# sinhvt3421/scann--material

Hardware: AMD Instinct MI355X
Metric: QM9 molecules/s forward (higher is better)
Workload: dtype f32 (projections: split-fp16 hi/lo operands, 3 v_mfma_f32_32x32x16_f16 per product, fp32 accumulate; everything else fp32)

## Files before the change

scann--material_amd/csrc/scann_edge_body.inc:

```
  _Float16* const sH = reinterpret_cast<_Float16*>(sTile);
  _Float16* const sL = sH + TEK * PLANE_STRIDE;
  float* const sK = reinterpret_cast<float*>(sTile);

  const int tid = threadIdx.x, lane = tid & 63, wave = tid >> 6;
  const int tix = SCANN_EDGE_TIX;
  const EdgeTile tile = a.tiles[tix];
  const int part = a.tile_part ? a.tile_part[tix] : -1;
  const int eb = tile.edge_begin, ne = tile.edge_end - eb, natom = tile.atom_end - tile.atom_begin;
  const int nem1 = ne > 0 ? ne - 1 : 0;
  const bool live = ne > 0;
  const int lrow = lane & 31, lh = lane >> 5;
  const int cbase = 32 * wave + 4 * lh;
  const int blk_jstride = 8 * ne;
  const auto blk_off = [&](int rt) __attribute__((always_inline)) {
    return ((unsigned)eb * D + ((unsigned)(8 * wave + lh) * ne + min(lrow + 32 * rt, nem1)) * 4) * 4;
  };

  STAMP(a.stamps, 0);
  STAMP_IF(a.stamps, 6, threadIdx.x == 0 && eb >= 0);
  STAMP_HWID(a.stamps, 14);
  STAMP_REAL(a.stamps, 12);
  WRegs<EX> wr;
  f16x8 fth[2], ftl[2];
  if (GUPD) {
    if (!FB) {
      load_whalf<EX>(wr, a.p.W2h, wave, lane, 0);
      __builtin_amdgcn_sched_barrier(0);
    }
  } else {
    load_wsplit<2>(a.p.Wfh, wave, lane, fth, ftl);
  }
  unsigned nboff[RT];
  int ctr[RT];
  float ewgt[RT] = {};
  const int32_t* const ecol = live ? a.edge_col : a.edge_offset;
  const int32_t* const erow = live ? a.edge_row : a.edge_offset;
#pragma unroll
  for (int rt = 0; rt < RT; ++rt) {
    const unsigned e4 = live ? (unsigned)(eb + min(lrow + 32 * rt, nem1)) * 4u : 0u;
    const int nbr = ld1i(ecol, e4), crw = ld1i(erow, e4);
    int nb = live ? nbr : 0;
    if (FB && a.species) nb = ld1i(a.species, (unsigned)nb * 4u);
    nboff[rt] = ((unsigned)nb * D + cbase) * 4;
    ctr[rt] = live ? crw - tile.atom_begin : 0;
    if (!GUPD) {
      const float wv = ld1f(live ? a.edge_weight : reinterpret_cast<const float*>(a.edge_offset), e4);
      ewgt[rt] = live ? wv : 0.f;
    }
  }
  const int voff = ld1i(a.edge_offset, (unsigned)(tile.atom_begin + min(tid, natom)) * 4u);
  STAMP_IF(a.stamps, 10, threadIdx.x == 0 && nboff[0] != 0xfffffff1u);
  const float bkc = a.p.bk[tid & (D - 1)];
  const float par0 = GUPD ? (tid < D ? a.p.lng_g : a.p.lng_b)[tid & (D - 1)] : a.p.bfg[tid & (D - 1)];
  const float par1 = (tid < D ? a.p.ln_g : a.p.ln_b)[tid & (D - 1)];
  float4 greg[RT][4];
  {
    const int r = tid >> 2, sub = tid & 3;
    const int rs = r < ne ? r : nem1;
    if (GUPD) {
      float4 p1reg[3];
#pragma unroll
      for (int i = 0; i < 3; ++i) {
        const int idx = tid + 256 * i, la = min(idx >> 5, natom - 1), c4 = idx & 31;
        const int arow = FB && a.species ? a.species[tile.atom_begin + la] : tile.atom_begin + la;
        p1reg[i] = ld4(a.P1, ((unsigned)arow * 32 + c4) * 16);
      }
      if (FB) {
        _Float16* const bH = reinterpret_cast<_Float16*>(sTile);
        _Float16* const bL = bH + TEK * BASIS_STRIDE;
        f16x8 bdh[2], bdl[2], bwh[2], bwl[2];
        load_wsplit<2>(a.basis.Wdh, wave, lane, bdh, bdl);
        load_wsplit<2>(a.basis.Wwh, wave, lane, bwh, bwl);
        {
          const float xd = ne > 0 ? a.dist[eb + rs] : 0.f, xw = ne > 0 ? a.edge_weight[eb + rs] : 0.f;
// ... 396 lines not shown
```

scann--material_amd/csrc/scann_forward.cpp:

```cpp
#include "scann_runtime.h"

namespace {

constexpr unsigned kTimingEventFlags = hipEventDisableSystemFence;

int ensure_debug(scann_handle* h, scann_dbatch* db) {
  const int L = h->cfg.n_attention;
  if (db->dbg_layers == L) return SCANN_OK;
  HIPCHK(h, cached_malloc((void**)&db->dbg_c, (size_t)(L + 1) * db->n_atom * D * 4));
  HIPCHK(h, cached_malloc((void**)&db->dbg_ctx, (size_t)std::max(L, 1) * db->n_atom * D * 4));
  if (h->cfg.g_update) HIPCHK(h, cached_malloc((void**)&db->dbg_g, (size_t)(L + 1) * std::max(db->n_edge, 1) * D * 4));
  db->dbg_layers = L;
  return SCANN_OK;
}

int ensure_outputs(scann_handle* h, scann_dbatch* db, bool infer) {
  db->out_layers = infer ? h->out_layers : 0;
  db->out_flags = infer ? h->out_flags : 0;
  db->out_attn = db->out_z = db->out_bf = nullptr;
  if (!db->out_layers && !db->out_flags) return SCANN_OK;
  const scann_config_t& c = h->cfg;
  const size_t n_attn = (size_t)__builtin_popcountll(db->out_layers) * db->n_edge * c.num_head;
  const size_t n_z = db->out_flags & SCANN_OUT_AFTER_LC ? (size_t)db->n_atom * c.global_dim : 0;
  const size_t n_bf = db->out_flags & SCANN_OUT_BF_PROPERTY ? (size_t)db->n_struct * c.dense_out : 0;
// ... 325 lines not shown
    }
#endif
    if (exact) {
      a.exact = 1;
      if (l > 0 && a.ffn) {
        const LayerParams& pp = W->layers[l - 1];
        a.Wf1h = reinterpret_cast<const _Float16*>(pp.Wf1p); a.Wf2h = reinterpret_cast<const _Float16*>(pp.Wf2p);
      }
      if (l < L) {
        const LayerParams& p = W->layers[l];
        a.WAh = reinterpret_cast<const _Float16*>(p.W1p); a.WBh = reinterpret_cast<const _Float16*>(p.W3p);
        a.WCh = reinterpret_cast<const _Float16*>(p.Wqp);
      } else {
        a.WAh = reinterpret_cast<const _Float16*>(W->head.Wap); a.WCh = reinterpret_cast<const _Float16*>(W->head.Wgqp);
        a.WDh = reinterpret_cast<const _Float16*>(W->head.Wgkp);
      }
    }
    if (!(species0 && l == 0)) launch_atom(a, s);
    if (tm) tm->mark(l < L ? 1 : 3);
    if (l == L) break;
    EdgeArgs ea{};
    ea.tiles = db->tiles; ea.n_tile = db->n_tile; ea.g_update = c.g_update; ea.tile_rows = db->tile_rows;
    ea.edge_offset = db->edge_offset; ea.edge_col = db->edge_col; ea.edge_row = db->edge_row;
    ea.geom = g_of(l); ea.geom_out = debug && c.g_update ? g_of(l + 1) : nullptr; ea.gd = b.gd; ea.edge_weight = db->weight;
    if (fuse_basis && l == 0) { ea.fuse_basis = 1; ea.dist = db->dist; ea.basis = W->basis; }
    ea.n_edge = db->n_edge;
    ea.geom_rows = fuse_basis ? 0 : 1;
    ea.geom_dead = (l == L - 1 && !debug) ? 1 : 0;
    ea.c = c_of(l); ea.P1 = b.P1; ea.P3 = b.P3; ea.q = keep ? db->keep_q + (size_t)l * nA_ : b.q; ea.ctx = ctx_of(l);
    ea.n_member = nm; ea.m_w = wst; ea.m_a = ea.m_r = ast;
    if (species0 && l == 0) { ea.species = db->atomic; ea.c = W->sp_c; ea.P1 = W->sp_P1; ea.P3 = W->sp_P3; ea.q = W->sp_q; ea.m_r = wst; }
    if (keep) {
      ea.keep_V = db->keep_V + (size_t)l * nE_; ea.keep_K = db->keep_K + (size_t)l * nE_;
      if (db->keep_T) ea.keep_T = db->keep_T + (size_t)l * nE_;
      if (db->keep_ang) ea.keep_ang = db->keep_ang + (size_t)l * nE_;
      db->kept = true;
    }
    ea.p = W->layers[l];
    if (exact) {
      ea.exact = 1;
      ea.p.W2h = reinterpret_cast<const _Float16*>(ea.p.W2p); ea.p.Wkh = reinterpret_cast<const _Float16*>(ea.p.Wkp);
    }
    ea.range_flag = rflag; ea.layer = l;
    const bool sample = !tm && !mc && !o.of_set && h->time_every > 0 && (h->time_count % h->time_every) == 0 && !(fuse_basis && l == 0) &&
                        !(ea.geom_dead && L > 2);
    hipEvent_t ev0 = nullptr, ev1 = nullptr;
    if (sample) {
      (void)hipEventCreateWithFlags(&ev0, kTimingEventFlags);
      (void)hipEventCreateWithFlags(&ev1, kTimingEventFlags);
      (void)hipEventRecord(ev0, s);
    }
    ea.tile_part = db->tile_part; ea.part_buf = b.part_buf;
    ea.xcd_remap = h->xcd_remap;
    ea.attn_out = o.outputs ? attn_out_of(h, db, l) : nullptr;
    if (tr && tr->attn_p > 0.f) {
      ea.attn_drop_p = tr->attn_p;
      ea.attn_drop_seed = tr->seed;
      ea.attn_drop_tag = DROP_TAG_ATTN + (unsigned)l;
    }
    if (mc && mc->p_attn > 0.f && db->n_edge > 0) {
      ea.attn_drop_p = mc->p_attn;
      ea.attn_drop_seed = mc->seed;
      ea.attn_drop_tag = DROP_TAG_ATTN + (unsigned)l;
      ea.mc_rows = mc->rows;
      ea.mc_t = mc->t;
    }
#ifdef SCANN_STAMPS
    if (!getenv("SCANN_STAMP_ATOM") && l == (getenv("SCANN_STAMP_LAYER") ? atoi(getenv("SCANN_STAMP_LAYER")) : L - 1)) {
      if (!db->stamps) HIPCHK(h, hipMalloc((void**)&db->stamps, (size_t)db->n_tile * 16 * sizeof(unsigned long long)));
      ea.stamps = db->stamps;
      db->n_stamp = db->n_tile;
    }
#endif
    launch_edge(ea, s);
    if (nm) launch_edge_merge_set(db->big_tab, db->n_big, b.part_buf, ea.q, ea.p.ln_g, ea.p.ln_b, ea.ctx, rflag, l, nm, ast, wst, s);
    else launch_edge_merge(db->big_tab, db->n_big, b.part_buf, ea.q, ea.p.ln_g, ea.p.ln_b, ea.ctx, rflag, l, s);
    if (ea.attn_out) launch_attn_merge(db->big_tab, db->n_big, b.part_buf, db->edge_offset, db->tile_rows, ea.attn_out, s);
    if (sample) {
      (void)hipEventRecord(ev1, s);
      h->time_ev.push_back(ev0);
      h->time_ev.push_back(ev1);
      h->time_edges.push_back(db->n_edge);
    }
    if (tm) tm->mark(2);
  }
  if (!tm && !mc && !o.of_set) h->time_count++;
  ReadoutArgs r{};
  r.mol_offset = db->mol_offset; r.n_struct = db->n_struct; r.max_atoms = db->max_atoms;
  r.gq = b.gq; r.gk = b.gk; r.use_ga_norm = c.use_ga_norm; r.relu_out = W->cfg.relu_out;
  for (int m = 1; m < nm; ++m) r.relu_out |= o.members[m]->cfg.relu_out << m;
  r.p = W->head; r.ga_attn = b.ga; r.y = b.y; r.bf_out = o.outputs ? db->out_bf : nullptr;
  r.n_member = nm; r.m_w = wst; r.m_a = ast; r.m_g = o.m_g; r.m_y = o.m_y;
  launch_readout(r, s);
  if (tm) tm->mark(3);
  HIPCHK(h, hipGetLastError());
  return SCANN_OK;
}

}

extern "C" {

int scann_forward_resident(scann_handle_t* h, scann_dbatch_t* db, int stream_slot) {
  if (!h || !db) return fail(h, SCANN_ERR_INVALID, "scann_forward_resident: null argument");
  HIPCHK(h, hipSetDevice(h->device));
  const int slot = ((stream_slot % h->nstream) + h->nstream) % h->nstream;
// ... 221 lines not shown
```

scann--material_amd/csrc/scann_internal.h:

```cpp
#pragma once
#include <hip/hip_runtime.h>
#include <stdint.h>

#include <string>
#include <vector>

namespace scann {

constexpr int D = 128;
constexpr int NHEAD = 8;
constexpr int HDIM = D / NHEAD;
constexpr int NG = 20;
constexpr int LDS_STRIDE = 132;
constexpr int TE_MAX = 64;
constexpr int TA = 64;
constexpr int TQ = 24;
constexpr int WPACK = D * D;
constexpr float WSCALE = 256.f;
constexpr float WMAX = 65504.f / WSCALE;

__host__ __device__ inline float drop_scale(unsigned long long seed, unsigned tag, size_t idx, float p) {
  unsigned long long z = seed + 0x9E3779B97F4A7C15ull * (idx + 1) + ((unsigned long long)tag << 48);
  z = (z ^ (z >> 30)) * 0xBF58476D1CE4E5B9ull;
  z = (z ^ (z >> 27)) * 0x94D049BB133111EBull;
// ... 84 lines not shown

void launch_basis(const BasisParams& p, const float* dist, const float* weight, int n_edge,
                  float* geom, hipStream_t s);
void launch_basis_raw(const float* cd, const float* dist, int n_edge, float* gd, hipStream_t s);

struct EmbedArgs {
  int32_t n_atom, emb_dim;
  const int32_t* atomic;
  const float* cgcnn;
  const float* ring;
  const float *emb;
  const float *We, *be;
  const float *Wr, *br;
  const float *Wde, *bde;
  float* c0;
};
void launch_embed(const EmbedArgs& a, hipStream_t s);

struct AtomArgs {
  const float* x;
  const int32_t* x_index;
  int32_t n_atom;
  int32_t ffn;
  const _Float16 *Wf1h, *Wf2h;
  const float *bf1, *bf2, *lnr_g, *lnr_b;
  float* c;
  float drop_p;
  uint32_t drop_tag;
  unsigned long long drop_seed;
  int32_t mode;
  const _Float16 *WAh, *WBh, *WCh, *WDh;
  const float *bA;
  const float *bC;
  const float *bD;
  float *oA, *oB, *oC;
  float *keep_pre1, *keep_H1, *keep_T2;
  float *keep_preA, *keep_z;
  unsigned long long* stamps;
  int32_t* range_flag;
  int32_t layer;
  int32_t exact;
  float* out_z;
  const McRow* mc_rows;
  uint32_t mc_t;
  int32_t n_member;
  int64_t m_w, m_x, m_o;
};
void launch_atom(const AtomArgs& a, hipStream_t s);

struct EdgeArgs {
  const EdgeTile* tiles;
  int32_t n_tile;
  int32_t xcd_remap;
  const int32_t* tile_part;
  float* part_buf;
  int32_t g_update;
  const int32_t* edge_offset;
  const int32_t* edge_col;
  const int32_t* edge_row;
  float* geom;
  float *keep_V, *keep_T, *keep_ang, *keep_K;
  float* geom_out;
  int32_t tile_rows;
  int32_t n_edge;
  int32_t geom_rows;
  int32_t geom_dead;
  const float* gd;
  const float* edge_weight;
  int32_t fuse_basis;
  const int32_t* species;
  const float* dist;
  BasisParams basis;
  const float *c, *P1, *P3, *q;
  float* ctx;
  float attn_drop_p;
  uint32_t attn_drop_tag;
  unsigned long long attn_drop_seed;
  unsigned long long* stamps;
  int32_t* range_flag;
  int32_t layer;
  int32_t exact;
  LayerParams p;
  float* attn_out;
  const McRow* mc_rows;
  uint32_t mc_t;
  int32_t n_member;
  int64_t m_w, m_r, m_a;
};
void launch_edge(const EdgeArgs& a, hipStream_t s);
void launch_attn_merge(const int32_t* big_tab, int n_big, const float* part_buf, const int32_t* edge_offset, int chunk, float* attn, hipStream_t s);
void launch_edge_merge(const int32_t* big_tab, int n_big, const float* part_buf, const float* q, const float* ln_g,
                       const float* ln_b, float* ctx, int32_t* range_flag, int layer, hipStream_t s);
void launch_edge_merge_set(const int32_t* big_tab, int n_big, const float* part_buf, const float* q, const float* ln_g, const float* ln_b,
                           float* ctx, int32_t* range_flag, int layer, int n_member, int64_t m_a, int64_t m_w, hipStream_t s);

struct GenSeg {
  const float* p;
  const int32_t* idx;
  int32_t w;
};
struct GenDenseArgs {
  GenSeg seg[3];
  int32_t n_seg;
  int32_t prod;
  const float* W;
  const float* b;
// ... 132 lines not shown
```

scann--material_amd/csrc/scann_kernels.hip:

```cpp
#include <algorithm>
#include <cstdlib>
#include <type_traits>
#include "scann_internal.h"
#include "scann_mma.h"

namespace scann {


__device__ __forceinline__ void mc_row_key(const AtomArgs& a, int atom, unsigned long long& seed, size_t& e) {
  const McRow m = a.mc_rows[atom];
  seed = mc_seed(a.drop_seed, a.mc_t, m.key);
  e = (size_t)(atom - m.a0) * D;
}
__device__ __forceinline__ float4 mc_drop4(unsigned long long seed, unsigned tag, size_t e, float p, float4 v) {
  v.x *= drop_scale(seed, tag, e, p);
  v.y *= drop_scale(seed, tag, e + 1, p);
  v.z *= drop_scale(seed, tag, e + 2, p);
  v.w *= drop_scale(seed, tag, e + 3, p);
  return v;
}
__device__ __forceinline__ float4 mc_keep4(uint32_t bits, float p, float4 v) {
  const float sc = 1.0f / (1.0f - p);
  v.x *= (bits & 1u) ? sc : 0.f;
  v.y *= (bits & 2u) ? sc : 0.f;
// ... 113 lines not shown
  } else {
    if (a.mode == 0) SCANN_ATOM_CASE(false, 0);
    else if (a.mode == 1) SCANN_ATOM_CASE(false, 1);
    else SCANN_ATOM_CASE(false, 2);
  }
#undef SCANN_ATOM_CASE
}


template <bool GUPD, int RT, bool FB = false, bool EX = false, bool KEEP = false, bool DEAD = false, bool ATTN = false, bool MC = false,
          bool SET = false>
__global__ __launch_bounds__(256, RT == 2 ? 3 : 4) void edge_kernel(EdgeArgs a) {
#pragma clang fp contract(off)
  static_assert(!FB || GUPD, "the fused basis exists for the g_update kernel only");
  static_assert(!(FB && EX), "the exact fallback runs the plain first layer");
  static_assert(!KEEP || (!FB && !EX && !DEAD), "the training forward runs the plain split-fp16 kernel and keeps every layer's geometry");
  static_assert(!DEAD || GUPD, "the base branch stores no geometry");
  static_assert(!(ATTN && KEEP), "the training forward returns no attention weights");
  static_assert(!MC || (!EX && !KEEP && !ATTN), "Monte Carlo dropout runs on the split-fp16 inference kernels and returns no attention weights");
  static_assert(!SET || (!EX && !KEEP && !ATTN && !MC), "a model set runs the split-fp16 inference kernels and returns no attention weights");
  constexpr int TEK = 32 * RT;
  constexpr bool BLK = GUPD && !EX && !KEEP;
  __shared__ __attribute__((aligned(16))) unsigned char sTile[2 * TEK * PLANE_STRIDE * 2];
  __shared__ __attribute__((aligned(16))) float sQ[TQ * LDS_STRIDE];
  __shared__ __attribute__((aligned(16))) float sE[NHEAD * (TEK + 1)];
#ifdef SCANN_DIAG_SE_ROWMAJOR
#define SE_STAT(w, r) (((r) * 4 + (w)) * 2)
#define SE_LOGIT(r, h) ((r) * NHEAD + (h))
#else
#define SE_STAT(w, r) (((w) * TEK + (r)) * 2)
#define SE_LOGIT(r, h) ((h) * (TEK + 1) + (r))
#endif
  __shared__ __attribute__((aligned(16))) float sPar[5 * D];
  __shared__ int sOff[TQ + 1];
#ifdef SCANN_DIAG_OCC2
  __shared__ float sDummy[7 * 1024];
  if (a.n_tile < 0) sDummy[threadIdx.x] = 1.f;
#endif
  static_assert(2 * TEK * PLANE_STRIDE * 2 >= TEK * LDS_STRIDE * (int)sizeof(float), "K tile must fit the plane buffer");
  int set_tix = 0;
  if constexpr (SET) {
    const int t = a.xcd_remap ? xcd_tile(blockIdx.x, gridDim.x) : blockIdx.x, m = t / a.n_tile;
    set_tix = t - m * a.n_tile;
    const int64_t w = (int64_t)m * a.m_w, r = (int64_t)m * a.m_r, x = (int64_t)m * a.m_a;
    a.p.W2h = set_member(a.p.W2h, w); a.p.Wkh = set_member(a.p.Wkh, w); a.p.Wfh = set_member(a.p.Wfh, w);
    a.p.bfg = set_member(a.p.bfg, w); a.p.bk = set_member(a.p.bk, w);
    a.p.lng_g = set_member(a.p.lng_g, w); a.p.lng_b = set_member(a.p.lng_b, w); a.p.ln_g = set_member(a.p.ln_g, w); a.p.ln_b = set_member(a.p.ln_b, w);
    a.basis.Wdh = set_member(a.basis.Wdh, w); a.basis.Wwh = set_member(a.basis.Wwh, w); a.basis.bd = set_member(a.basis.bd, w);
    a.basis.bw = set_member(a.basis.bw, w); a.basis.cd = set_member(a.basis.cd, w); a.basis.cw = set_member(a.basis.cw, w);
    a.c = set_member(a.c, r); a.P1 = set_member(a.P1, r); a.P3 = set_member(a.P3, r); a.q = set_member(a.q, r);
    a.geom = set_member(a.geom, x); a.ctx = set_member(a.ctx, x); a.part_buf = set_member(a.part_buf, x);
  }
#define SCANN_EDGE_TIX (SET ? set_tix : a.xcd_remap ? xcd_tile(blockIdx.x, gridDim.x) : blockIdx.x)
#include "scann_edge_body.inc"
#undef SCANN_EDGE_TIX
#undef SE_STAT
#undef SE_LOGIT
#ifdef SCANN_DIAG_TAILWAIT
  __builtin_amdgcn_s_waitcnt(0);
  __syncthreads();
#endif
}

template <bool SET = false>
__global__ __launch_bounds__(128) void edge_merge_kernel(const int32_t* __restrict__ big_tab, const float* __restrict__ part_buf,
                                                         const float* __restrict__ q, const float* __restrict__ ln_g,
                                                         const float* __restrict__ ln_b, float* __restrict__ ctx,
                                                         int32_t* __restrict__ range_flag, int layer, int n_big, int64_t m_a, int64_t m_w) {
  __shared__ float sRed[2][2];
  unsigned bix = blockIdx.x;
  if constexpr (SET) {
    const unsigned m = blockIdx.x / (unsigned)n_big;
    bix = blockIdx.x - m * (unsigned)n_big;
    part_buf = set_member(part_buf, (int64_t)m * m_a); q = set_member(q, (int64_t)m * m_a); ctx = set_member(ctx, (int64_t)m * m_a);
    ln_g = set_member(ln_g, (int64_t)m * m_w); ln_b = set_member(ln_b, (int64_t)m * m_w);
  }
  const int c = threadIdx.x, atom = big_tab[3 * bix], s0 = big_tab[3 * bix + 1], ns = big_tab[3 * bix + 2];
  const float* pb = part_buf + (size_t)s0 * 3 * D + c;
  float M = -INFINITY;
  for (int i = 0; i < ns; ++i) M = fmaxf(M, pb[(size_t)i * 3 * D]);
  float S = 0.f, X = 0.f;
  for (int i = 0; i < ns; ++i) {
    const float wgt = fast_exp(pb[(size_t)i * 3 * D] - M);
    S += pb[(size_t)i * 3 * D + D] * wgt;
    X += pb[(size_t)i * 3 * D + 2 * D] * wgt;
  }
  const float t = X * __builtin_amdgcn_rcpf(S) + q[(size_t)atom * D + c];
  float s = t;
#pragma unroll
  for (int o = 1; o < 64; o <<= 1) s += __shfl_xor(s, o);
  if ((c & 63) == 0) sRed[0][c >> 6] = s;
  __syncthreads();
  const float mean = (sRed[0][0] + sRed[0][1]) * (1.0f / D);
  const float d = t - mean;
  float v = d * d;
#pragma unroll
  for (int o = 1; o < 64; o <<= 1) v += __shfl_xor(v, o);
  if ((c & 63) == 0) sRed[1][c >> 6] = v;
  __syncthreads();
  if (!(sRed[1][0] + sRed[1][1] < RANGE_FINITE) && c == 0) flag_range(range_flag, 2, layer);
  const float rstd = ln_rstd((sRed[1][0] + sRed[1][1]) * (1.0f / D));
  ctx[(size_t)atom * D + c] = ln_apply(t, rstd, -mean * rstd, ln_g[c], ln_b[c]);
}

void launch_edge_merge(const int32_t* big_tab, int n_big, const float* part_buf, const float* q, const float* ln_g,
                       const float* ln_b, float* ctx, int32_t* range_flag, int layer, hipStream_t s) {
  if (n_big > 0)
    hipLaunchKernelGGL(edge_merge_kernel<false>, dim3(n_big), dim3(128), 0, s, big_tab, part_buf, q, ln_g, ln_b, ctx, range_flag, layer, n_big,
                       (int64_t)0, (int64_t)0);
}
void launch_edge_merge_set(const int32_t* big_tab, int n_big, const float* part_buf, const float* q, const float* ln_g, const float* ln_b,
                           float* ctx, int32_t* range_flag, int layer, int n_member, int64_t m_a, int64_t m_w, hipStream_t s) {
  if (n_big > 0 && n_member > 0)
    hipLaunchKernelGGL(edge_merge_kernel<true>, dim3(n_big * n_member), dim3(128), 0, s, big_tab, part_buf, q, ln_g, ln_b, ctx, range_flag, layer,
// ... 14 lines not shown
    const float mi = pb[(size_t)(n / chunk) * 3 * D];
    float* const w = attn + (size_t)(e0 + n) * NHEAD + h;
    *w = *w * fast_exp(mi - M) * __builtin_amdgcn_rcpf(S);
  }
}

void launch_attn_merge(const int32_t* big_tab, int n_big, const float* part_buf, const int32_t* edge_offset, int chunk, float* attn, hipStream_t s) {
  if (n_big > 0 && attn) hipLaunchKernelGGL(attn_merge_kernel, dim3(n_big), dim3(256), 0, s, big_tab, part_buf, edge_offset, chunk, attn);
}

__global__ void edge_row_kernel(const int32_t* __restrict__ edge_offset, int n_atom, int32_t* __restrict__ edge_row, int32_t* __restrict__ zero_word) {
  const int a = blockIdx.x * blockDim.x + threadIdx.x;
  if (a == 0 && zero_word) *zero_word = 0;
  if (a >= n_atom) return;
  for (int e = edge_offset[a]; e < edge_offset[a + 1]; ++e) edge_row[e] = a;
}
void launch_edge_row(const int32_t* edge_offset, int n_atom, int32_t* edge_row, hipStream_t s, int32_t* zero_word) {
  if (n_atom > 0 || zero_word)
    hipLaunchKernelGGL(edge_row_kernel, dim3(std::max(1, (n_atom + 255) / 256)), dim3(256), 0, s, edge_offset, n_atom, edge_row, zero_word);
}

__global__ __launch_bounds__(256) void pack_padded_kernel(PackPaddedArgs a) {
  const int bm = blockIdx.x * blockDim.x + threadIdx.x;
  if (bm >= a.B * a.M) return;
  const int row = a.row_of[bm];
  if (row < 0) return;
  const int z = a.atomic[bm];
  int bad = (z < 0 || z >= a.n_species) ? 2 : 0;
  a.out_atomic[row] = bad ? 0 : z;
  const int b0 = (bm / a.M) * a.M;
  int e = a.edge_offset[row];
  const size_t base = (size_t)bm * a.N;
  for (int n = 0; n < a.N; ++n) {
    const bool on = a.mask_size == 1 ? static_cast<const uint8_t*>(a.neighbor_mask)[base + n] != 0
                                     : (static_cast<const uint32_t*>(a.neighbor_mask)[base + n] & 0x7fffffffu) != 0;
    if (!on) continue;
    const int tgt = a.neighbors[base + n];
    const int r = (tgt >= 0 && tgt < a.M) ? a.row_of[b0 + tgt] : -1;
    if (r < 0) bad |= 1;
    a.out_col[e] = r < 0 ? row : r;
    a.out_dist[e] = a.dist[base + n];
    a.out_weight[e] = a.weight[base + n];
    ++e;
  }
  if (bad) atomicOr(a.flag, bad);
}
void launch_pack_padded(const PackPaddedArgs& a, hipStream_t s) {
  const int n = a.B * a.M;
  if (n > 0) hipLaunchKernelGGL(pack_padded_kernel, dim3((n + 255) / 256), dim3(256), 0, s, a);
}

void launch_edge(const EdgeArgs& a, hipStream_t s) {
  if (a.n_tile <= 0) return;
  const dim3 grid(a.n_tile * std::max(a.n_member, 1)), block(256);
  const bool keep = !a.exact && (a.geom_rows || a.keep_V || a.keep_T || a.keep_ang || a.keep_K || a.attn_drop_p > 0.f);
  const bool dead = a.g_update && a.geom_dead && !keep;
#define SCANN_EDGE_GO(...) hipLaunchKernelGGL((edge_kernel<__VA_ARGS__>), grid, block, 0, s, a)
#define SCANN_EDGE_ROWS(G, ...)                                             \
  do {                                                                      \
    if (a.tile_rows == 32) SCANN_EDGE_GO(G, 1, __VA_ARGS__);                \
    else SCANN_EDGE_GO(G, 2, __VA_ARGS__);                                  \
  } while (0)
  if (a.n_member > 0) {
    if (!a.g_update) SCANN_EDGE_ROWS(false, false, false, false, false, false, false, true);
    else if (a.fuse_basis) SCANN_EDGE_ROWS(true, true, false, false, false, false, false, true);
    else if (a.geom_dead) SCANN_EDGE_ROWS(true, false, false, false, true, false, false, true);
    else SCANN_EDGE_ROWS(true, false, false, false, false, false, false, true);
  } else if (a.mc_rows && a.attn_drop_p > 0.f) {
    if (!a.g_update) SCANN_EDGE_ROWS(false, false, false, false, false, false, true);
    else if (a.fuse_basis) SCANN_EDGE_ROWS(true, true, false, false, false, false, true);
    else if (a.geom_dead) SCANN_EDGE_ROWS(true, false, false, false, true, false, true);
    else SCANN_EDGE_ROWS(true, false, false, false, false, false, true);
  } else if (a.exact && a.attn_out) {
    if (!a.g_update) SCANN_EDGE_ROWS(false, false, true, false, false, true);
    else if (dead) SCANN_EDGE_ROWS(true, false, true, false, true, true);
    else SCANN_EDGE_ROWS(true, false, true, false, false, true);
  } else if (a.exact) {
    if (!a.g_update) SCANN_EDGE_ROWS(false, false, true, false, false);
    else if (dead) SCANN_EDGE_ROWS(true, false, true, false, true);
    else SCANN_EDGE_ROWS(true, false, true, false, false);
  } else if (a.attn_out) {
    if (!a.g_update) SCANN_EDGE_ROWS(false, false, false, false, false, true);
    else if (a.fuse_basis) SCANN_EDGE_ROWS(true, true, false, false, false, true);
    else if (a.geom_dead) SCANN_EDGE_ROWS(true, false, false, false, true, true);
    else SCANN_EDGE_ROWS(true, false, false, false, false, true);
  } else if (keep) {
    if (a.g_update) SCANN_EDGE_ROWS(true, false, false, true, false);
    else SCANN_EDGE_ROWS(false, false, false, true, false);
  } else if (!a.g_update) {
    SCANN_EDGE_ROWS(false, false, false, false, false);
  } else if (a.fuse_basis) {
    SCANN_EDGE_ROWS(true, true, false, false, false);
  } else {
    if (dead) SCANN_EDGE_ROWS(true, false, false, false, true);
    else SCANN_EDGE_ROWS(true, false, false, false, false);
  }
#undef SCANN_EDGE_ROWS
#undef SCANN_EDGE_GO
}


__global__ __launch_bounds__(256) void basis_kernel(BasisParams p, const float* __restrict__ dist,
                                                    const float* __restrict__ weight, int n_edge,
                                                    float* __restrict__ geom) {
#pragma clang fp contract(off)
  __shared__ __attribute__((aligned(16))) _Float16 sH[64 * BASIS_STRIDE];
  __shared__ __attribute__((aligned(16))) _Float16 sL[64 * BASIS_STRIDE];
  const int tid = threadIdx.x, lane = tid & 63, wave = tid >> 6;
  const int lrow = lane & 31, lh = lane >> 5, cbase = 32 * wave + 4 * lh;
  const int e0 = blockIdx.x * 64;
  const int ne = min(64, n_edge - e0);
  f16x8 bdh[2], bdl[2], bwh[2], bwl[2];
  load_wsplit<2>(p.Wdh, wave, lane, bdh, bdl);
  load_wsplit<2>(p.Wwh, wave, lane, bwh, bwl);
  float4 bd[4], bw[4];
#pragma unroll
  for (int j = 0; j < 4; ++j) {
    bd[j] = *reinterpret_cast<const float4*>(p.bd + cbase + 8 * j);
    bw[j] = *reinterpret_cast<const float4*>(p.bw + cbase + 8 * j);
  }
  {
    const int r = tid >> 2, sub = tid & 3;
    const int rs = min(r, ne - 1);
    const float xd = dist[e0 + rs], xw = weight[e0 + rs];
    f16x8 gh[2], gl[2];
#pragma unroll
    for (int i = 0; i < 8; ++i) {
      const int k = 8 * sub + i;
      const float cdk = p.cd[min(k, NG - 1)], cwk = p.cw[min(k, NG - 1)];
      const float vd = (k < NG && r < ne) ? gauss_fast(xd, cdk) : 0.f, vw = (k < NG && r < ne) ? gauss_fast(xw, cwk) : 0.f;
      gh[0][i] = (_Float16)vd; gl[0][i] = (_Float16)(vd - (float)gh[0][i]);
      gh[1][i] = (_Float16)vw; gl[1][i] = (_Float16)(vw - (float)gh[1][i]);
    }
    *reinterpret_cast<f16x8*>(sH + r * BASIS_STRIDE + 8 * sub) = gh[0];
    *reinterpret_cast<f16x8*>(sL + r * BASIS_STRIDE + 8 * sub) = gl[0];
    *reinterpret_cast<f16x8*>(sH + r * BASIS_STRIDE + 32 + 8 * sub) = gh[1];
    *reinterpret_cast<f16x8*>(sL + r * BASIS_STRIDE + 32 + 8 * sub) = gl[1];
  }
  __syncthreads();
  f32x16 accd[2], accw[2];
  mma_split<2, true, BASIS_STRIDE>(sH, sL, bdh, bdl, lane, accd);
  mma_split<2, true, BASIS_STRIDE>(sH + 32, sL + 32, bwh, bwl, lane, accw);
  constexpr float WINV = 1.0f / WSCALE;
// ... 260 lines not shown
```

scann--material_amd/csrc/scann_runtime.cpp:

```cpp
#include "scann_runtime.h"

#include <mutex>

namespace {

struct BlockCache {
  std::multimap<size_t, void*> free_blocks;
  std::map<void*, size_t> size_of;
  size_t cached_bytes = 0;
};
std::map<int, BlockCache> g_block_cache;
std::mutex g_block_mu;
constexpr size_t BLOCK_CACHE_LIMIT = (size_t)16 << 30;
thread_local std::string g_create_error;

std::vector<WeightSpec> build_specs(const scann_config_t& c) {
  std::vector<WeightSpec> s;
  const int64_t d = c.local_dim, dg = c.global_dim, dout = c.dense_out, emb = c.embedding_dim;
  if (c.feature_cgcnn) {
    s.push_back({"embed_atom/kernel", 92, emb});
    s.push_back({"embed_atom/bias", emb, 0});
  } else {
    s.push_back({"embed_atom/embeddings", c.n_atoms, emb});
  }
// ... 188 lines not shown
    for (int s = 0; s < ks; ++s)
      for (int lane = 0; lane < 64; ++lane)
        for (int j = 0; j < 8; ++j) {
          const int k = 16 * s + 8 * (lane >> 5) + j;
          const float x = k < k_real ? WSCALE * W[(size_t)k * ld + 32 * w + (lane & 31)] : 0.f;
          const uint16_t hi = f32_to_f16_bits(x);
          const uint16_t lo = f32_to_f16_bits(x - f16_bits_to_f32(hi));
          const size_t base = ((size_t)(w * ks + s) * 2) * 64 * 8 + (size_t)lane * 8 + j;
          out[base] = hi;
          out[base + 64 * 8] = lo;
        }
}

}

extern "C" {

int scann_abi_version(void) { return SCANN_ABI_VERSION; }

int scann_device_count(void) {
  int n = 0;
  if (hipGetDeviceCount(&n) != hipSuccess) return 0;
  return n;
}

const char* scann_last_error(const scann_handle_t* h) { return h ? h->err.c_str() : g_create_error.c_str(); }

int scann_create(const scann_config_t* cfg, int device_id, scann_handle_t** out) {
  if (!cfg || !out) return fail(nullptr, SCANN_ERR_INVALID, "scann_create: null argument");
  *out = nullptr;
  if (cfg->n_gauss != NG) return fail(nullptr, SCANN_ERR_UNSUPPORTED, "scann_create: 20 Gaussians (custom_layers.py:39-53 as called by scann_model.py:378,384)");
  const bool generic = cfg->local_dim != D || cfg->global_dim != D || cfg->dense_out != D || cfg->num_head != NHEAD ||
                       (getenv("SCANN_GENERIC") && atoi(getenv("SCANN_GENERIC")));
  if (generic) {
    if (cfg->local_dim <= 0 || cfg->num_head <= 0 || cfg->global_dim <= 0 || cfg->dense_out <= 0 || cfg->local_dim % cfg->num_head != 0)
      return fail(nullptr, SCANN_ERR_INVALID, "scann_create: local_dim must be a positive multiple of num_head (attention.py:170-173), global_dim and dense_out positive");
    if (cfg->local_dim > 1024 || cfg->global_dim > 1024 || cfg->dense_out > 1024 || cfg->embedding_dim > 1024)
      return fail(nullptr, SCANN_ERR_UNSUPPORTED, "scann_create: widths above 1024 are not implemented");
  } else if (cfg->embedding_dim + (cfg->use_ring ? 10 : 0) > 160) {
    return fail(nullptr, SCANN_ERR_UNSUPPORTED, "scann_create: embedding_dim (+10 ring features) must be <= 160");
  }
  if (cfg->n_atoms <= 0 || cfg->embedding_dim <= 0 || cfg->n_attention < 0 || !(cfg->gaussian_d > 0))
    return fail(nullptr, SCANN_ERR_INVALID, "scann_create: bad hyper-parameter");
  int ndev = 0;
  if (hipGetDeviceCount(&ndev) != hipSuccess || ndev <= 0)
    return fail(nullptr, SCANN_ERR_NO_DEVICE, "scann_create: no HIP device visible (this library has no CPU fallback)");
  if (device_id < 0 || device_id >= ndev) return fail(nullptr, SCANN_ERR_NO_DEVICE, "scann_create: device_id out of range");
  scann_handle* h = new scann_handle();
  h->cfg = *cfg;
  h->generic = generic;
  h->device = device_id;
  h->specs = build_specs(*cfg);
  if (const char* xr = getenv("SCANN_XCD_REMAP")) h->xcd_remap = atoi(xr) != 0;
  if (const char* fb = getenv("SCANN_FUSE_BASIS")) h->fuse_basis = atoi(fb) != 0;
  if (const char* st = getenv("SCANN_SPECIES_TABLES")) h->species_tables = atoi(st) != 0;
  if (const char* sg = getenv("SCANN_STRICT_RANGE")) h->strict_range = atoi(sg) != 0;
  if (const char* fe = getenv("SCANN_EXACT")) h->force_exact = atoi(fe) != 0;
  {
    hipDeviceProp_t prop;
    if (hipGetDeviceProperties(&prop, device_id) == hipSuccess && prop.multiProcessorCount > 0) h->n_cu = prop.multiProcessorCount;
  }
  if (const char* ns = getenv("SCANN_STREAMS")) h->nstream = std::min(MAX_STREAM, std::max(1, atoi(ns)));
  if (hipSetDevice(device_id) != hipSuccess) {
    delete h;
    return fail(nullptr, SCANN_ERR_HIP, "scann_create: hipSetDevice failed");
  }
  if (hipHostMalloc((void**)&h->range_flag, 128, hipHostMallocDefault) != hipSuccess) {
    delete h;
    return fail(nullptr, SCANN_ERR_HIP, "scann_create: hipHostMalloc failed");
  }
  for (int i = 0; i < 32; ++i) h->range_flag[i] = 0;
  for (int i = 0; i < h->nstream; ++i) {
    if (hipStreamCreateWithFlags(&h->streams[i], hipStreamNonBlocking) != hipSuccess) {
      delete h;
      return fail(nullptr, SCANN_ERR_HIP, "scann_create: hipStreamCreate failed");
    }
  }
  *out = h;
  return SCANN_OK;
}

void scann_destroy(scann_handle_t* h) {
  if (!h) return;
  (void)hipSetDevice(h->device);
  (void)hipDeviceSynchronize();
  for (int i = 0; i < MAX_STREAM; ++i)
    if (h->streams[i]) (void)hipStreamDestroy(h->streams[i]);
  if (h->d_weights) (void)hipFree(h->d_weights);
  for (scann_handle::DlStage& st : h->dl_stage)
    if (st.p) (void)hipHostFree(st.p);
  if (h->g_weights) (void)hipFree(h->g_weights);
  if (h->g_centres) (void)hipFree(h->g_centres);
  if (h->g_WT) (void)hipFree(h->g_WT);
  if (h->d_gt_descs) (void)hipFree(h->d_gt_descs);
  if (h->sp_c) (void)hipFree(h->sp_c);
  for (scann_handle::Stage& st : h->stage) {
    if (st.p) (void)hipHostFree(st.p);
    if (st.ev) (void)hipEventDestroy(st.ev);
  }
  if (h->copy_stream) (void)hipStreamDestroy(h->copy_stream);
  for (void* q : {(void*)h->t_master, (void*)h->t_grad, (void*)h->t_m, (void*)h->t_v, (void*)h->t_l2, (void*)h->t_descs, (void*)h->ig_grad})
    if (q) (void)hipFree(q);
  if (h->comm) ncclCommDestroy(h->comm);
  if (h->train_aux && !h->train_aux_borrowed) (void)hipStreamDestroy(h->train_aux);
  if (h->h_stat) (void)hipHostFree(h->h_stat);
  if (h->range_flag) (void)hipHostFree(h->range_flag);
// ... 358 lines not shown
```

scann--material_amd/csrc/scann_runtime.h:

```cpp
#pragma once
#include "../../include/scann_hip.h"
#include "scann_internal.h"
#include "scann_train.h"

#include <rccl/rccl.h>

#include <algorithm>
#include <cmath>
#include <cstdlib>
#include <cstring>
#include <map>
#include <memory>
#include <string>
#include <vector>

using namespace scann;

namespace scann {

constexpr int MAX_STREAM = 16;

hipError_t cached_malloc(void** p, size_t bytes);
void cached_free(void* p);
void cache_release(int dev);
// ... 36 lines not shown
  float *keep_preA = nullptr, *keep_z = nullptr;
  std::vector<float*> tE;
  float *rep = nullptr, *dpre = nullptr, *dy = nullptr, *targets = nullptr, *dlut = nullptr;
  float* wpart = nullptr;
  size_t wpart_floats = 0;
  float* det_part = nullptr;
  size_t det_floats = 0;
  double* sse = nullptr;
  char* ig = nullptr;
  size_t ig_bytes = 0;
  float drop_p = 0.f, attn_p = 0.f;
  unsigned long long seed = 0;
  GenKeep gen;
  ~scann_train_ws() {
    cached_free(arena);
    cached_free(det_part);
    cached_free(ig);
    cached_free(gen.arena);
    cached_free(gen.barena);
  }
};

struct Timer;
struct ModelSet;
void free_models(ModelSet* ms);

struct McState {
  const McRow* rows;
  unsigned long long seed;
  uint32_t t;
  float p_drop, p_attn;
};

}

struct scann_handle {
  scann_config_t cfg{};
  int device = 0;
  std::string err;
  hipStream_t streams[MAX_STREAM]{};
  int nstream = 2;
  std::vector<WeightSpec> specs;
  bool loaded = false;
  bool debug = false;
  uint64_t out_layers = 0;
  int32_t out_flags = 0;
  int tile_atoms = TQ;
  int n_cu = 256;
  int time_every = 0;
  int64_t time_count = 0;
  std::vector<hipEvent_t> time_ev;
  std::vector<int> time_edges;
  int xcd_remap = 1;
  int fuse_basis = 1;
  int species_tables = 1;
  bool generic = false;
  float* g_weights = nullptr;
  float* g_centres = nullptr;
  std::map<std::string, int64_t> g_off;
  std::vector<GenTransDesc> gt_descs;
  GenTransDesc* d_gt_descs = nullptr;
  std::map<std::string, int64_t> gt_off;
  float* g_WT = nullptr;
  int gt_max = 0;
  bool weights_exact = false;
  bool force_exact = false;
  bool strict_range = false;
  int64_t exact_reruns = 0;
  float* d_weights = nullptr;
  std::vector<LayerParams> layers;
  HeadParams head{};
  BasisParams basis{};
  const float* lut = nullptr;
  float *sp_c = nullptr, *sp_P1 = nullptr, *sp_P3 = nullptr, *sp_q = nullptr;
  bool sp_dirty = true;
  const float* cd = nullptr;
  EmbedArgs embed{};
  std::vector<float> host_master;
  std::vector<int64_t> spec_off;
  std::vector<RepackDesc> descs;
  size_t arena_floats = 0, o_lut = 0, o_emb = 0, o_Wde = 0, o_bde = 0;
  struct LayerT {
    const float *W1T, *W2T, *W3T, *WqT, *WkT, *Wf1T, *Wf2T;
    const _Float16 *W1Th, *W2Th, *W3Th, *WqTh, *WkTh, *Wf1Th, *Wf2Th;
  };
  std::vector<LayerT> layersT;
  const float *WaT = nullptr, *WgqT = nullptr, *WgkT = nullptr;
  const _Float16* WaTh = nullptr;
  float *t_master = nullptr, *t_grad = nullptr, *t_m = nullptr, *t_v = nullptr, *t_l2 = nullptr;
  RepackDesc* t_descs = nullptr;
  float* ig_grad = nullptr;
  int64_t t_step = 0;
  float attn_drop_p = 0.f;
  bool deterministic = false;
  ncclComm_t comm = nullptr;
  double* h_stat = nullptr;
  float* h_targets[3] = {nullptr, nullptr, nullptr};
  size_t h_targets_cap[3] = {0, 0, 0};
  hipEvent_t step_ev[2] = {nullptr, nullptr};
  int64_t step_begun = 0, step_ended = 0;
  bool grads_zeroed = false;
  struct Stage { char* p = nullptr; size_t cap = 0; hipEvent_t ev = nullptr; bool used = false; };
  static constexpr int N_STAGE = 8;
  Stage stage[N_STAGE];
  int stage_next = 0;
  struct PadScratch { std::vector<int32_t> gidx, at, mol, eoff, col; std::vector<float> dist, wgt, ga; };
// ... 137 lines not shown
```

Baseline: 2.022 million.

## Process edge tiles in pairs per block to cut per-block launch overhead

Adds an edge_pair_kernel that loops over two consecutive edge tiles per workgroup for the bulk of tiles, with the remainder handled one tile per block. The aim is to amortise block startup costs such as weight-register loads and kernarg reads, and to cut wave-launch overhead across the grid. The pair count is rounded to a multiple of three blocks per CU. In exchange, per-block work becomes serial and the added inter-tile __syncthreads may reduce latency hiding. It also relies on the asm barriers (fresh_tid, fresh_edge_args) to keep register pressure in check. The path is enabled by default for 64-row tiles with g_update.

```diff
diff --git a/scann--material_amd/csrc/scann_edge_body.inc b/scann--material_amd/csrc/scann_edge_body.inc
--- a/scann--material_amd/csrc/scann_edge_body.inc
+++ b/scann--material_amd/csrc/scann_edge_body.inc
@@ -2,7 +2,7 @@
   _Float16* const sL = sH + TEK * PLANE_STRIDE;
   float* const sK = reinterpret_cast<float*>(sTile);
 
-  const int tid = threadIdx.x, lane = tid & 63, wave = tid >> 6;
+  const int tid = SCANN_EDGE_TID, lane = tid & 63, wave = tid >> 6;
   const int tix = SCANN_EDGE_TIX;
   const EdgeTile tile = a.tiles[tix];
   const int part = a.tile_part ? a.tile_part[tix] : -1;
@@ -16,10 +16,11 @@
     return ((unsigned)eb * D + ((unsigned)(8 * wave + lh) * ne + min(lrow + 32 * rt, nem1)) * 4) * 4;
   };
 
-  STAMP(a.stamps, 0);
+  STAMP_IF(a.stamps, 0, threadIdx.x == 0 && SCANN_EDGE_ENTRY);
   STAMP_IF(a.stamps, 6, threadIdx.x == 0 && eb >= 0);
   STAMP_HWID(a.stamps, 14);
-  STAMP_REAL(a.stamps, 12);
+  STAMP_IF(a.stamps, 15, threadIdx.x == 0 && !SCANN_EDGE_ENTRY);
+  if (SCANN_EDGE_ENTRY) STAMP_REAL(a.stamps, 12);
   WRegs<EX> wr;
   f16x8 fth[2], ftl[2];
   if (GUPD) {
diff --git a/scann--material_amd/csrc/scann_forward.cpp b/scann--material_amd/csrc/scann_forward.cpp
--- a/scann--material_amd/csrc/scann_forward.cpp
+++ b/scann--material_amd/csrc/scann_forward.cpp
@@ -401,6 +401,10 @@
     }
     ea.tile_part = db->tile_part; ea.part_buf = b.part_buf;
     ea.xcd_remap = h->xcd_remap;
+    if (h->edge_pair && db->tile_rows == 64) {
+      const int slots = 3 * h->n_cu;
+      ea.n_pair = (db->n_tile / slots) * slots / 2;
+    }
     ea.attn_out = o.outputs ? attn_out_of(h, db, l) : nullptr;
     if (tr && tr->attn_p > 0.f) {
       ea.attn_drop_p = tr->attn_p;
diff --git a/scann--material_amd/csrc/scann_internal.h b/scann--material_amd/csrc/scann_internal.h
--- a/scann--material_amd/csrc/scann_internal.h
+++ b/scann--material_amd/csrc/scann_internal.h
@@ -160,6 +160,7 @@
   const EdgeTile* tiles;
   int32_t n_tile;
   int32_t xcd_remap;
+  int32_t n_pair;
   const int32_t* tile_part;
   float* part_buf;
   int32_t g_update;
diff --git a/scann--material_amd/csrc/scann_kernels.hip b/scann--material_amd/csrc/scann_kernels.hip
--- a/scann--material_amd/csrc/scann_kernels.hip
+++ b/scann--material_amd/csrc/scann_kernels.hip
@@ -189,7 +189,11 @@
     a.geom = set_member(a.geom, x); a.ctx = set_member(a.ctx, x); a.part_buf = set_member(a.part_buf, x);
   }
 #define SCANN_EDGE_TIX (SET ? set_tix : a.xcd_remap ? xcd_tile(blockIdx.x, gridDim.x) : blockIdx.x)
+#define SCANN_EDGE_TID threadIdx.x
+#define SCANN_EDGE_ENTRY true
 #include "scann_edge_body.inc"
+#undef SCANN_EDGE_ENTRY
+#undef SCANN_EDGE_TID
 #undef SCANN_EDGE_TIX
 #undef SE_STAT
 #undef SE_LOGIT
@@ -197,6 +201,54 @@
   __builtin_amdgcn_s_waitcnt(0);
   __syncthreads();
 #endif
+}
+
+__device__ __forceinline__ int fresh_tid() {
+  int t = threadIdx.x;
+  asm volatile("" : "+v"(t));
+  return t;
+}
+__device__ __forceinline__ const __attribute__((address_space(4))) EdgeArgs& fresh_edge_args() {
+  auto p = __builtin_amdgcn_kernarg_segment_ptr();
+  asm volatile("" : "+s"(p));
+  return *(const __attribute__((address_space(4))) EdgeArgs*)p;
+}
+template <bool FB, bool DEAD>
+__global__ __launch_bounds__(256, 3) void edge_pair_kernel(EdgeArgs args) {
+#pragma clang fp contract(off)
+  constexpr bool GUPD = true, EX = false, KEEP = false, ATTN = false, MC = false, BLK = true;
+  constexpr int RT = 2, TEK = 32 * RT;
+  __shared__ __attribute__((aligned(16))) unsigned char sTile[2 * TEK * PLANE_STRIDE * 2];
+  __shared__ __attribute__((aligned(16))) float sQ[TQ * LDS_STRIDE];
+  __shared__ __attribute__((aligned(16))) float sE[NHEAD * (TEK + 1)];
+#define SE_STAT(w, r) (((w) * TEK + (r)) * 2)
+#define SE_LOGIT(r, h) ((h) * (TEK + 1) + (r))
+  __shared__ __attribute__((aligned(16))) float sPar[5 * D];
+  __shared__ int sOff[TQ + 1];
+  const int b = blockIdx.x, np = args.n_pair;
+  int pair_tix, pair_end;
+  if (b < np) {
+    pair_tix = 2 * (args.xcd_remap ? xcd_tile(b, np) : b);
+    pair_end = pair_tix + 2;
+  } else {
+    pair_tix = 2 * np + (args.xcd_remap ? xcd_tile(b - np, (int)gridDim.x - np) : b - np);
+    pair_end = pair_tix + 1;
+  }
+#define SCANN_EDGE_TIX pair_tix
+#define SCANN_EDGE_TID fresh_tid()
+#define SCANN_EDGE_ENTRY ((pair_tix & 1) == 0 || pair_tix >= 2 * args.n_pair)
+#pragma unroll 1
+  for (;;) {
+    const auto& a = fresh_edge_args();
+#include "scann_edge_body.inc"
+    if (++pair_tix == pair_end) break;
+    __syncthreads();
+  }
+#undef SCANN_EDGE_ENTRY
+#undef SCANN_EDGE_TID
+#undef SCANN_EDGE_TIX
+#undef SE_STAT
+#undef SE_LOGIT
 }
 
 template <bool SET = false>
@@ -317,7 +369,7 @@
 
 void launch_edge(const EdgeArgs& a, hipStream_t s) {
   if (a.n_tile <= 0) return;
-  const dim3 grid(a.n_tile * std::max(a.n_member, 1)), block(256);
+  dim3 grid(a.n_tile * std::max(a.n_member, 1)), block(256);
   const bool keep = !a.exact && (a.geom_rows || a.keep_V || a.keep_T || a.keep_ang || a.keep_K || a.attn_drop_p > 0.f);
   const bool dead = a.g_update && a.geom_dead && !keep;
 #define SCANN_EDGE_GO(...) hipLaunchKernelGGL((edge_kernel<__VA_ARGS__>), grid, block, 0, s, a)
@@ -354,6 +406,11 @@
     else SCANN_EDGE_ROWS(false, false, false, true, false);
   } else if (!a.g_update) {
     SCANN_EDGE_ROWS(false, false, false, false, false);
+  } else if (a.n_pair > 0 && a.tile_rows == 64) {
+    grid = dim3(a.n_tile - a.n_pair);
+    if (a.fuse_basis) hipLaunchKernelGGL((edge_pair_kernel<true, false>), grid, block, 0, s, a);
+    else if (dead) hipLaunchKernelGGL((edge_pair_kernel<false, true>), grid, block, 0, s, a);
+    else hipLaunchKernelGGL((edge_pair_kernel<false, false>), grid, block, 0, s, a);
   } else if (a.fuse_basis) {
     SCANN_EDGE_ROWS(true, true, false, false, false);
   } else {
diff --git a/scann--material_amd/csrc/scann_runtime.cpp b/scann--material_amd/csrc/scann_runtime.cpp
--- a/scann--material_amd/csrc/scann_runtime.cpp
+++ b/scann--material_amd/csrc/scann_runtime.cpp
@@ -264,6 +264,7 @@
   h->device = device_id;
   h->specs = build_specs(*cfg);
   if (const char* xr = getenv("SCANN_XCD_REMAP")) h->xcd_remap = atoi(xr) != 0;
+  if (const char* ep = getenv("SCANN_EDGE_PAIR")) h->edge_pair = atoi(ep) != 0;
   if (const char* fb = getenv("SCANN_FUSE_BASIS")) h->fuse_basis = atoi(fb) != 0;
   if (const char* st = getenv("SCANN_SPECIES_TABLES")) h->species_tables = atoi(st) != 0;
   if (const char* sg = getenv("SCANN_STRICT_RANGE")) h->strict_range = atoi(sg) != 0;
diff --git a/scann--material_amd/csrc/scann_runtime.h b/scann--material_amd/csrc/scann_runtime.h
--- a/scann--material_amd/csrc/scann_runtime.h
+++ b/scann--material_amd/csrc/scann_runtime.h
@@ -112,6 +112,7 @@
   std::vector<hipEvent_t> time_ev;
   std::vector<int> time_edges;
   int xcd_remap = 1;
+  int edge_pair = 1;
   int fuse_basis = 1;
   int species_tables = 1;
   bool generic = false;
```

New measurement: 1.949 million. 3.6% lower.
